# wg-perception/tod

Hardware: AMD Instinct MI355X
Metric: frames/sec @ 640x480, 1M-descriptor DB; achieved HBM GB/s on BF-matcher (higher is better)
Workload: dtype fp4 (+-1) x fp4 -> f32 on the matrix cores (exact integers), f32 in the verifier

## Files before the change

tod_amd/csrc/match_fp4rows.h:

```cpp

__global__ __launch_bounds__(kBlock) void expand_rows_fp4_kernel(const uint32_t* __restrict__ db, uint32_t n_steps, uint4* __restrict__ out) {
  const uint32_t s = blockIdx.x, m = threadIdx.x >> 6, l = threadIdx.x & 63u;
  if (s >= n_steps) return;
  const Fp4Consts kc = fp4_consts();
  const mfma_i32x8 e = expand_word(db[(size_t)fp4_rows_src_row(s, l) * kWords + fp4_rows_src_word(m, l)], kc);
  *reinterpret_cast<uint4*>(reinterpret_cast<char*>(out) + fp4_rows_offset(s, m, l)) =
      uint4{(uint32_t)e[0], (uint32_t)e[1], (uint32_t)e[2], (uint32_t)e[3]};
}
static_assert(kBlock == 256, "expand_rows_fp4_kernel: one workgroup = the 4 x 64 fragments of a step");

typedef uint32_t fp4_u32x4 __attribute__((ext_vector_type(4)));
struct Fp4StepLoader {
  __amdgpu_buffer_rsrc_t copy;
  uint32_t step0, n_steps, lane_off;
  __device__ __forceinline__ Fp4StepLoader(const uint4* p, uint32_t copy_bytes, uint32_t s0, uint32_t n, uint32_t lane)
      : copy(__builtin_amdgcn_make_buffer_rsrc(const_cast<uint4*>(p), 0, (int)copy_bytes, 0x00020000)), step0(s0), n_steps(n),
        lane_off((uint32_t)fp4_rows_offset(0, 0, lane)) {}
  template <bool M_SCALAR>
  __device__ __forceinline__ mfma_i32x8 load(uint32_t step, uint32_t m) const {
    const uint32_t step_off = (uint32_t)fp4_rows_offset(step0 + min(step, n_steps - 1u), M_SCALAR ? m : 0u, 0);
    const fp4_u32x4 v = __builtin_amdgcn_raw_buffer_load_b128(copy, (int)(lane_off + (M_SCALAR ? 0u : m * kFp4FragBytes)), (int)step_off, 0);
    return mfma_i32x8{(int)v.x, (int)v.y, (int)v.z, (int)v.w, 0, 0, 0, 0};
  }
};

template <int K, int SPLIT>
__device__ __forceinline__ void fp4rows_block_test_part(mfma_f32x16& acc, const Fp4Row& rows, const Fp4Row& q, float& thr, float& thrp,
                                                        uint32_t r_lane, uint32_t n_lim, uint32_t (&best)[K], uint32_t& n_pass) {
  if (__builtin_expect(__builtin_amdgcn_ballot_w64(block_reaches<true, false>(acc, thrp)) == 0ull, 1)) return;
  ++n_pass;
#pragma unroll
  for (int s = SPLIT; s < 4; ++s) acc = __builtin_amdgcn_mfma_scale_f32_32x32x64_f8f6f4(rows.s[s], q.s[s], acc, 4, 4, 0, 0, 0, 0);
  mfma_block_test<K, false, true>(acc, thr, r_lane, n_lim, best);
  thrp = thr - 64.f * (float)(4 - SPLIT);
}

template <int N>
struct Fp4Frags { mfma_i32x8 s[N]; };
template <int N>
__device__ __forceinline__ mfma_f32x16 dot_frags(const Fp4Frags<N>& a, const Fp4Frags<N>& b) {
  mfma_f32x16 acc = {0.f, 0.f, 0.f, 0.f, 0.f, 0.f, 0.f, 0.f, 0.f, 0.f, 0.f, 0.f, 0.f, 0.f, 0.f, 0.f};
#pragma unroll
  for (int s = 0; s < N; ++s) acc = __builtin_amdgcn_mfma_scale_f32_32x32x64_f8f6f4(a.s[s], b.s[s], acc, 4, 4, 0, 0, 0, 0);
  return acc;
}
__device__ __forceinline__ uint4 load_query_packed(const uint32_t* __restrict__ q, uint32_t qi, uint32_t nq, uint32_t h) {
  return *reinterpret_cast<const uint4*>(q + (size_t)(qi < nq ? qi : nq - 1u) * kWords + 4u * h);
}
__device__ __forceinline__ uint32_t packed_word(const uint4& p, int m) { return m == 0 ? p.x : m == 1 ? p.y : m == 2 ? p.z : p.w; }

template <int K, int SPLIT>
__device__ __forceinline__ void fp4rows_block_test_part(mfma_f32x16& acc, const Fp4StepLoader& rows, uint32_t own_step,
                                                        const uint32_t* __restrict__ q, uint32_t qi, uint32_t nq, uint32_t h,
                                                        const Fp4Consts& kc, float& thr, float& thrp, uint32_t r_lane, uint32_t n_lim,
                                                        uint32_t (&best)[K], uint32_t& n_pass) {
  if (__builtin_expect(__builtin_amdgcn_ballot_w64(block_reaches<true, false>(acc, thrp)) == 0ull, 1)) return;
  ++n_pass;
  asm volatile("" : "+v"(qi));
  mfma_i32x8 tail[4 - SPLIT];
#pragma unroll
  for (int s = SPLIT; s < 4; ++s) tail[s - SPLIT] = rows.template load<true>(own_step, s);
  const uint4 p = load_query_packed(q, qi, nq, h);
#pragma unroll
  for (int s = SPLIT; s < 4; ++s)
    acc = __builtin_amdgcn_mfma_scale_f32_32x32x64_f8f6f4(tail[s - SPLIT], expand_word(packed_word(p, s), kc), acc, 4, 4, 0, 0, 0, 0);
  mfma_block_test<K, false, true>(acc, thr, r_lane, n_lim, best);
  asm("" : "+v"(thr));
  thrp = thr - 64.f * (float)(4 - SPLIT);
}

template <int K, int QT, bool MASK, bool IMAX, int SPLIT = 0>
__device__ __forceinline__ void fp4rows_step(const Fp4Row& a, Fp4Row& a_next, const Fp4StepLoader& rows, uint32_t next_step,
                                             const Fp4Row (&qb)[QT], float (&thr)[QT], float (&thrp)[QT], uint32_t (&best)[QT][K],
                                             mfma_f32x16& acc_even, mfma_f32x16& acc_odd, uint32_t r_lane, uint32_t n_lim, uint32_t& n_pass) {
  constexpr bool HALF = SPLIT != 0;
  constexpr int kEarly = HALF ? SPLIT : 4;
  static_assert(!(HALF && MASK) && !(HALF && !IMAX) && QT >= 4, "split blocks: unmasked steps, integer maximum; >= 4 query blocks");
  static_assert(SPLIT == 0 || SPLIT == 2 || SPLIT == 3, "2 or 3 of the 4 MFMAs first");
#pragma unroll
  for (int t = 0; t < QT; ++t) {
    if (HALF) { if (t & 1) acc_odd = dot_part0<HALF ? SPLIT : 2>(a, qb[t]); else acc_even = dot_part0<HALF ? SPLIT : 2>(a, qb[t]); }
    else { if (t & 1) acc_odd = dot_block(a, qb[t]); else acc_even = dot_block(a, qb[t]); }
    if (t == 0) {
#pragma unroll
      for (int m = 0; m < kEarly; ++m) a_next.s[m] = rows.template load<!HALF>(next_step, m);
    }
    if (t == 1) {
#pragma unroll
      for (int m = kEarly; m < 4; ++m) a_next.s[m] = rows.template load<!HALF>(next_step, m);
    }
    if (HALF) {
      if (t == 0) fp4rows_block_test_part<K, HALF ? SPLIT : 2>(acc_odd, a_next, qb[QT - 1], thr[QT - 1], thrp[QT - 1], r_lane - 32u, n_lim, best[QT - 1], n_pass);
      else fp4rows_block_test_part<K, HALF ? SPLIT : 2>((t & 1) ? acc_even : acc_odd, a, qb[t - 1], thr[t - 1], thrp[t - 1], r_lane, n_lim, best[t - 1], n_pass);
    } else {
      if (t == 0) mfma_block_test<K, MASK, IMAX>(acc_odd, thr[QT - 1], r_lane - 32u, n_lim, best[QT - 1]);
      else mfma_block_test<K, MASK, IMAX>((t & 1) ? acc_even : acc_odd, thr[t - 1], r_lane, n_lim, best[t - 1]);
    }
  }
}

template <int K, int QT, int SPLIT>
__device__ __forceinline__ void fp4rows_split_step(const Fp4Frags<SPLIT>& a, Fp4Frags<SPLIT>& a_next, const Fp4StepLoader& rows, uint32_t step,
                                                   const Fp4Frags<SPLIT> (&qh)[QT], const uint32_t* __restrict__ q, uint32_t q0c, uint32_t nq,
                                                   uint32_t h, const Fp4Consts& kc, float (&thr)[QT], float (&thrp)[QT],
                                                   uint32_t (&best)[QT][K], mfma_f32x16& acc_even, mfma_f32x16& acc_odd, uint32_t r_lane,
                                                   uint32_t n_lim, uint32_t& n_pass) {
  static_assert(SPLIT == 2 || SPLIT == 3, "2 or 3 of the 4 MFMAs first");
  static_assert(QT >= 4 && QT % 2 == 0, "the pending block alternates between two accumulators");
#pragma unroll
  for (int t = 0; t < QT; ++t) {
    if (t & 1) acc_odd = dot_frags(a, qh[t]); else acc_even = dot_frags(a, qh[t]);
    if (t == 0) {
#pragma unroll
      for (int m = 0; m < SPLIT; ++m) a_next.s[m] = rows.template load<false>(step + 1u, m);
    }
    if (t == 0) fp4rows_block_test_part<K, SPLIT>(acc_odd, rows, step - 1u, q, q0c + 32u * (QT - 1), nq, h, kc, thr[QT - 1], thrp[QT - 1], r_lane - 32u, n_lim, best[QT - 1], n_pass);
    else fp4rows_block_test_part<K, SPLIT>((t & 1) ? acc_even : acc_odd, rows, step, q, q0c + 32u * (t - 1), nq, h, kc, thr[t - 1], thrp[t - 1], r_lane, n_lim, best[t - 1], n_pass);
  }
}

struct PairConsts {
  mfma_f32x16 magic;
  int scale_one, scale_field;
  int bias;
};
__device__ __forceinline__ PairConsts pair_consts(uint32_t cut) {
  PairConsts pk;
  const float m = PairPack::magic(cut);
#pragma unroll
  for (int i = 0; i < 16; ++i) pk.magic[i] = m;
  asm volatile("v_mov_b32 %0, %1" : "=v"(pk.scale_one) : "n"(PairPack::kScaleOne));
  asm volatile("v_mov_b32 %0, %1" : "=v"(pk.scale_field) : "n"(PairPack::kScaleField));
  pk.bias = PairPack::bias(cut);
  return pk;
}
__device__ __forceinline__ void dot_pair(mfma_f32x16& acc, const Fp4Frags<2>& a, const Fp4Frags<2>& qa, const Fp4Frags<2>& qb, const PairConsts& pk) {
  acc = __builtin_amdgcn_mfma_scale_f32_32x32x64_f8f6f4(a.s[0], qa.s[0], pk.magic, 4, 4, 0, 0, 0, 0);
  acc = __builtin_amdgcn_mfma_scale_f32_32x32x64_f8f6f4(a.s[1], qa.s[1], acc, 4, 4, 0, 0, 0, 0);
  acc = __builtin_amdgcn_mfma_scale_f32_32x32x64_f8f6f4(a.s[0], qb.s[0], acc, 4, 4, 0, pk.scale_field, 0, pk.scale_one);
  acc = __builtin_amdgcn_mfma_scale_f32_32x32x64_f8f6f4(a.s[1], qb.s[1], acc, 4, 4, 0, pk.scale_field, 0, pk.scale_one);
  asm volatile("" : "+v"(acc));
}
__device__ __forceinline__ uint32_t pair_or(const mfma_f32x16& acc) {
  uint32_t g[5];
#pragma unroll
  for (int j = 0; j < 5; ++j) {
    g[j] = (uint32_t)__float_as_int(acc[3 * j]) | (uint32_t)__float_as_int(acc[3 * j + 1]) | (uint32_t)__float_as_int(acc[3 * j + 2]);
    asm("" : "+v"(g[j]));
  }
  return (g[0] | g[1] | g[2]) | (g[3] | g[4] | (uint32_t)__float_as_int(acc[15]));
}
template <int K, int FIELD>
__device__ __forceinline__ void fp4rows_pair_complete(const mfma_f32x16& packed, int bias, const Fp4StepLoader& rows, uint32_t own_step,
                                                      const uint32_t* __restrict__ q, uint32_t qi, uint32_t nq, uint32_t h, const Fp4Consts& kc,
                                                      float& thr, uint32_t r_lane, uint32_t n_lim, uint32_t (&best)[K], uint32_t& n_pass) {
  ++n_pass;
  asm volatile("" : "+v"(qi));
  mfma_f32x16 acc;
#pragma unroll
  for (int i = 0; i < 16; ++i) acc[i] = (float)PairPack::unpack((uint32_t)__float_as_int(packed[i]), FIELD, bias);
  mfma_i32x8 tail[2];
#pragma unroll
  for (int s = 2; s < 4; ++s) tail[s - 2] = rows.template load<true>(own_step, s);
  const uint4 p = load_query_packed(q, qi, nq, h);
#pragma unroll
  for (int s = 2; s < 4; ++s)
    acc = __builtin_amdgcn_mfma_scale_f32_32x32x64_f8f6f4(tail[s - 2], expand_word(packed_word(p, s), kc), acc, 4, 4, 0, 0, 0, 0);
  mfma_block_test<K, false, true>(acc, thr, r_lane, n_lim, best);
  asm("" : "+v"(thr));
}
template <int K>
__device__ __forceinline__ void fp4rows_pair_test(const mfma_f32x16& acc, const PairConsts& pk, const Fp4StepLoader& rows, uint32_t own_step,
                                                  const uint32_t* __restrict__ q, uint32_t qi, uint32_t nq, uint32_t h, const Fp4Consts& kc,
                                                  float& thr_a, float& thr_b, uint32_t r_lane, uint32_t n_lim, uint32_t (&best_a)[K],
                                                  uint32_t (&best_b)[K], uint32_t& n_pass) {
  const uint32_t o = pair_or(acc);
  if (__builtin_expect(__builtin_amdgcn_ballot_w64((o & PairPack::kFlagMask) != 0u) == 0ull, 1)) return;
  if (__builtin_amdgcn_ballot_w64((o & PairPack::kFlagA) != 0u) != 0ull)
    fp4rows_pair_complete<K, 0>(acc, pk.bias, rows, own_step, q, qi, nq, h, kc, thr_a, r_lane, n_lim, best_a, n_pass);
  if (__builtin_amdgcn_ballot_w64((o & PairPack::kFlagB) != 0u) != 0ull)
    fp4rows_pair_complete<K, 1>(acc, pk.bias, rows, own_step, q, qi + 32u, nq, h, kc, thr_b, r_lane, n_lim, best_b, n_pass);
}
template <int K, int QT, int PH>
__device__ __forceinline__ void fp4rows_pair_step(const Fp4Frags<2>& a, Fp4Frags<2>& a_next, const Fp4StepLoader& rows, uint32_t step,
                                                  const Fp4Frags<2> (&qh)[QT], const uint32_t* __restrict__ q, uint32_t q0c, uint32_t nq,
                                                  uint32_t h, const Fp4Consts& kc, const PairConsts& pk, float (&thr)[QT],
                                                  uint32_t (&best)[QT][K], mfma_f32x16& acc_even, mfma_f32x16& acc_odd, uint32_t r_lane,
                                                  uint32_t n_lim, uint32_t& n_pass) {
  static_assert(QT >= 4 && QT % 2 == 0, "whole pairs; the pending pair alternates between two accumulators");
  constexpr int NP = QT / 2;
#pragma unroll
  for (int j = 0; j < NP; ++j) {
    const bool odd = ((NP * PH + j) & 1) != 0;
    dot_pair(odd ? acc_odd : acc_even, a, qh[2 * j], qh[2 * j + 1], pk);
    if (j == 0) {
#pragma unroll
      for (int m = 0; m < 2; ++m) a_next.s[m] = rows.template load<false>(step + 1u, m);
    }
    constexpr int kLast = NP - 1;
    if (j == 0) fp4rows_pair_test<K>(odd ? acc_even : acc_odd, pk, rows, step - 1u, q, q0c + 64u * kLast, nq, h, kc, thr[2 * kLast], thr[2 * kLast + 1], r_lane - 32u, n_lim, best[2 * kLast], best[2 * kLast + 1], n_pass);
    else fp4rows_pair_test<K>(odd ? acc_even : acc_odd, pk, rows, step, q, q0c + 64u * (j - 1), nq, h, kc, thr[2 * j - 2], thr[2 * j - 1], r_lane, n_lim, best[2 * j - 2], best[2 * j - 1], n_pass);
  }
}

template <int K, int QT, int SPLIT>
__device__ __forceinline__ void fp4rows_split_masked_step(const Fp4Row& a, const Fp4Frags<SPLIT> (&qh)[QT], const uint32_t (&qtail)[QT][4 - SPLIT],
                                                          const Fp4Consts& kc, float (&thr)[QT], uint32_t (&best)[QT][K],
                                                          mfma_f32x16& acc_even, mfma_f32x16& acc_odd, uint32_t r_lane, uint32_t n_lim) {
#pragma unroll
  for (int t = 0; t < QT; ++t) {
    Fp4Frags<SPLIT> ah;
#pragma unroll
    for (int s = 0; s < SPLIT; ++s) ah.s[s] = a.s[s];
    mfma_f32x16 acc = dot_frags(ah, qh[t]);
#pragma unroll
    for (int s = SPLIT; s < 4; ++s) acc = __builtin_amdgcn_mfma_scale_f32_32x32x64_f8f6f4(a.s[s], expand_word(qtail[t][s - SPLIT], kc), acc, 4, 4, 0, 0, 0, 0);
    if (t & 1) acc_odd = acc; else acc_even = acc;
    if (t == 0) mfma_block_test<K, true, true>(acc_odd, thr[QT - 1], r_lane - 32u, n_lim, best[QT - 1]);
    else mfma_block_test<K, true, true>((t & 1) ? acc_even : acc_odd, thr[t - 1], r_lane, n_lim, best[t - 1]);
  }
}

#ifndef TOD_K4X_STATIC_PRIO
#define TOD_K4X_STATIC_PRIO 1
#endif
template <int K, int QT, int MODE>
__global__ __launch_bounds__(kBlock, 2) void hamming_topk_fp4rows(const uint4* __restrict__ rows_fp4,
                                                                  const uint32_t* __restrict__ q, uint32_t n_rows,
                                                                  uint32_t nq, uint32_t nq_pad, uint32_t rows_per_tile,
                                                                  uint32_t n_tiles, uint32_t n_qw, uint32_t n_qw64,
                                                                  uint32_t blocks_per_xcd, uint32_t tiles_per_xcd, uint32_t cut,
                                                                  uint32_t share_period,
                                                                  uint32_t* __restrict__ part, uint32_t* bound,
                                                                  uint8_t* __restrict__ stored, uint32_t* half_stats) {
  static_assert(QT == 4 || QT == 6, "four or six query blocks per wave: with eight the fragments of two steps do not fit beside them");
  constexpr bool IMAX = MODE >= 1;
  constexpr int HALF = MODE == 4 ? 2 : (MODE >= 2 ? MODE : 0);
  constexpr float kPartOff = HALF ? 64.f * (float)(4 - HALF) : 0.f;
  const uint32_t xcd = blockIdx.x & 7u, slot = blockIdx.x >> 3;
  uint32_t tile, qw;
  if (tiles_per_xcd) {
    const uint32_t local = __builtin_amdgcn_readfirstlane(slot * kWavesPerBlock + (threadIdx.x >> 6));
    if (local >= tiles_per_xcd * n_qw) return;
    tile = xcd * tiles_per_xcd + local / n_qw; qw = local % n_qw;
  } else {
    const uint32_t vblock = xcd * blocks_per_xcd + slot;
    const uint32_t item = __builtin_amdgcn_readfirstlane(vblock * kWavesPerBlock + (threadIdx.x >> 6));
    tile = item / n_qw; qw = item % n_qw;
  }
  if (tile >= n_tiles) return;
  const uint32_t lane = threadIdx.x & 63u, c = lane & 31u, h = lane >> 5;
  const uint32_t q0 = qw * (32u * QT);

  const Fp4Consts kc = fp4_consts();
  constexpr bool TAILS = HALF == 2;
  constexpr bool PAIRS = MODE == 2;
  constexpr int NF = TAILS ? HALF : 4;
  using Frags = typename std::conditional<TAILS, Fp4Frags<NF>, Fp4Row>::type;
  Frags qb[QT];
  uint32_t best[QT][K];
  float thr[QT], thrp[QT];
#pragma unroll
  for (int t = 0; t < QT; ++t) {
    if constexpr (TAILS) {
      const uint4 p = load_query_packed(q, q0 + 32u * t + c, nq, h);
#pragma unroll
      for (int m = 0; m < NF; ++m) qb[t].s[m] = expand_word(packed_word(p, m), kc);
    } else {
      load_query_block(q, q0 + 32u * t + c, nq, h, qb[t], kc);
    }
#pragma unroll
    for (int j = 0; j < K; ++j) best[t][j] = 0xFFFFFFFFu;
    thr[t] = thr_of_limit(cut);
    if constexpr (!PAIRS) thrp[t] = thr[t] - kPartOff;
  }

  const uint32_t row0 = tile * rows_per_tile;
  const uint32_t n_local = min(n_rows, row0 + rows_per_tile) - row0;
  const uint32_t n_full = n_local / 32u, n_steps = (n_local + 31u) / 32u;
  const Fp4StepLoader rows(rows_fp4, (uint32_t)fp4_rows_bytes(n_rows), row0 / 32u, n_steps, lane);
  Frags a0, a1;
#pragma unroll
  for (int m = 0; m < NF; ++m) a0.s[m] = rows.template load<false>(0, m);
  a1 = a0;
  mfma_f32x16 acc_even, acc_odd;
  PairConsts pk;
  if constexpr (PAIRS) { pk = pair_consts(cut); acc_odd = pk.magic; }
  else {
#pragma unroll
    for (int i = 0; i < 16; ++i) acc_odd[i] = kNoBlock;
  }
  uint32_t seen[QT];
#pragma unroll
  for (int t = 0; t < QT; ++t) seen[t] = 0xFFFFFFFFu;
  uint32_t next_share = 2u, step = 0, n_pass = 0;
  if (TOD_K4X_STATIC_PRIO && HALF == 2 && QT == 6 && ((slot >> 5) & 1u)) __builtin_amdgcn_s_setprio(1);
  for (; step + 2u <= n_full; step += 2u) {
    if constexpr (PAIRS) {
      fp4rows_pair_step<K, QT, 0>(a0, a1, rows, step, qb, q, q0 + c, nq, h, kc, pk, thr, best, acc_even, acc_odd, lane_row_base(step, h), n_local, n_pass);
      fp4rows_pair_step<K, QT, 1>(a1, a0, rows, step + 1u, qb, q, q0 + c, nq, h, kc, pk, thr, best, acc_even, acc_odd, lane_row_base(step, h) + 32u, n_local, n_pass);
    } else if constexpr (TAILS) {
      fp4rows_split_step<K, QT, NF>(a0, a1, rows, step, qb, q, q0 + c, nq, h, kc, thr, thrp, best, acc_even, acc_odd, lane_row_base(step, h), n_local, n_pass);
      fp4rows_split_step<K, QT, NF>(a1, a0, rows, step + 1u, qb, q, q0 + c, nq, h, kc, thr, thrp, best, acc_even, acc_odd, lane_row_base(step, h) + 32u, n_local, n_pass);
    } else {
      fp4rows_step<K, QT, false, IMAX, HALF>(a0, a1, rows, step + 1u, qb, thr, thrp, best, acc_even, acc_odd, lane_row_base(step, h), n_local, n_pass);
      fp4rows_step<K, QT, false, IMAX, HALF>(a1, a0, rows, step + 2u, qb, thr, thrp, best, acc_even, acc_odd, lane_row_base(step, h) + 32u, n_local, n_pass);
    }
    if (step + 2u >= next_share) {
      next_share += share_period;
      exchange_bounds<K, QT>(bound, q0, c, nq, best, seen, thr, [](uint32_t limit) { return thr_of_limit(limit); },
                             [&](int t) { if constexpr (!PAIRS) thrp[t] = thr[t] - kPartOff; });
    }
  }
  if constexpr (TAILS) {
    if (step > 0u) {
      if constexpr (PAIRS)
        fp4rows_pair_test<K>(acc_odd, pk, rows, step - 1u, q, q0 + c + 32u * (QT - 2), nq, h, kc, thr[QT - 2], thr[QT - 1], lane_row_base(step - 1u, h), n_local, best[QT - 2], best[QT - 1], n_pass);
      else
        fp4rows_block_test_part<K, NF>(acc_odd, rows, step - 1u, q, q0 + c + 32u * (QT - 1), nq, h, kc, thr[QT - 1], thrp[QT - 1], lane_row_base(step - 1u, h), n_local, best[QT - 1], n_pass);
#pragma unroll
      for (int i = 0; i < 16; ++i) acc_odd[i] = kNoBlock;
      if (lane == 0 && half_stats) { atomicAdd(half_stats, n_pass); atomicAdd(half_stats + 1, step * (uint32_t)QT); }
    }
    if (step < n_steps) {
      uint32_t qtail[QT][4 - NF];
#pragma unroll
      for (int t = 0; t < QT; ++t) {
        const uint4 p = load_query_packed(q, q0 + 32u * t + c, nq, h);
#pragma unroll
        for (int m = NF; m < 4; ++m) qtail[t][m - NF] = packed_word(p, m);
      }
      Fp4Row a, a_next;
#pragma unroll
      for (int m = 0; m < NF; ++m) a.s[m] = a0.s[m];
#pragma unroll
      for (int m = NF; m < 4; ++m) a.s[m] = rows.template load<false>(step, m);
      for (; step < n_steps; ++step) {
#pragma unroll
        for (int m = 0; m < 4; ++m) a_next.s[m] = rows.template load<false>(step + 1u, m);
        fp4rows_split_masked_step<K, QT, NF>(a, qb, qtail, kc, thr, best, acc_even, acc_odd, lane_row_base(step, h), n_local);
        a = a_next;
      }
    }
  } else {
    if (HALF && step > 0u) {
      fp4rows_block_test_part<K, HALF ? HALF : 2>(acc_odd, a1, qb[QT - 1], thr[QT - 1], thrp[QT - 1], lane_row_base(step - 1u, h), n_local, best[QT - 1], n_pass);
#pragma unroll
      for (int i = 0; i < 16; ++i) acc_odd[i] = kNoBlock;
      if (lane == 0 && half_stats) { atomicAdd(half_stats, n_pass); atomicAdd(half_stats + 1, step * (uint32_t)QT); }
    }
    for (; step < n_steps; ++step) {
      fp4rows_step<K, QT, true, IMAX>(a0, a1, rows, step + 1u, qb, thr, thrp, best, acc_even, acc_odd, lane_row_base(step, h), n_local, n_pass);
      a0 = a1;
    }
  }
  mfma_block_test<K, true, IMAX>(acc_odd, thr[QT - 1], lane_row_base(n_steps - 1u, h), n_local, best[QT - 1]);
  store_tile_lists<K, QT>(best, tile, q0, nq, nq_pad, n_qw64, lane, c, h, part, stored);
}
```

Baseline: 23820.

## Move cross-tile bound exchange into rare pair-complete path for PAIRS variant

For the paired-query path, the periodic exchange_bounds call in the main loop is removed. Each query's global bound is instead read and atomically lowered only inside fp4rows_pair_complete, which runs when a candidate passes the packed test. The row-base lane offset is now recomputed there instead of being passed through every step call. This cuts periodic synchronisation and register pressure in the hot loop, at the cost of fresher thresholds arriving only on rare completion events, so pruning may be weaker between events.

```diff
diff --git a/tod_amd/csrc/match_fp4rows.h b/tod_amd/csrc/match_fp4rows.h
--- a/tod_amd/csrc/match_fp4rows.h
+++ b/tod_amd/csrc/match_fp4rows.h
@@ -153,9 +153,13 @@
 template <int K, int FIELD>
 __device__ __forceinline__ void fp4rows_pair_complete(const mfma_f32x16& packed, int bias, const Fp4StepLoader& rows, uint32_t own_step,
                                                       const uint32_t* __restrict__ q, uint32_t qi, uint32_t nq, uint32_t h, const Fp4Consts& kc,
-                                                      float& thr, uint32_t r_lane, uint32_t n_lim, uint32_t (&best)[K], uint32_t& n_pass) {
+                                                      float& thr, uint32_t n_lim, uint32_t (&best)[K], uint32_t& n_pass, uint32_t* bound) {
   ++n_pass;
   asm volatile("" : "+v"(qi));
+  asm volatile("" : "+v"(h));
+  const uint32_t r_lane = lane_row_base(own_step, h);
+  uint32_t* my_bound = bound + (qi < nq ? qi : nq - 1u);
+  const uint32_t seen = __hip_atomic_load(my_bound, __ATOMIC_RELAXED, __HIP_MEMORY_SCOPE_AGENT);
   mfma_f32x16 acc;
 #pragma unroll
   for (int i = 0; i < 16; ++i) acc[i] = (float)PairPack::unpack((uint32_t)__float_as_int(packed[i]), FIELD, bias);
@@ -166,27 +170,30 @@
 #pragma unroll
   for (int s = 2; s < 4; ++s)
     acc = __builtin_amdgcn_mfma_scale_f32_32x32x64_f8f6f4(tail[s - 2], expand_word(packed_word(p, s), kc), acc, 4, 4, 0, 0, 0, 0);
+  if (seen != 0xFFFFFFFFu) thr = fmaxf(thr, thr_of_limit(seen + 1u));
   mfma_block_test<K, false, true>(acc, thr, r_lane, n_lim, best);
+  const uint32_t worst_d = best[K - 1] >> kLocalBits;
+  if (worst_d < kNoLimit && worst_d < seen) atomicMin(my_bound, worst_d);
   asm("" : "+v"(thr));
 }
 template <int K>
 __device__ __forceinline__ void fp4rows_pair_test(const mfma_f32x16& acc, const PairConsts& pk, const Fp4StepLoader& rows, uint32_t own_step,
                                                   const uint32_t* __restrict__ q, uint32_t qi, uint32_t nq, uint32_t h, const Fp4Consts& kc,
-                                                  float& thr_a, float& thr_b, uint32_t r_lane, uint32_t n_lim, uint32_t (&best_a)[K],
-                                                  uint32_t (&best_b)[K], uint32_t& n_pass) {
+                                                  float& thr_a, float& thr_b, uint32_t n_lim, uint32_t (&best_a)[K],
+                                                  uint32_t (&best_b)[K], uint32_t& n_pass, uint32_t* bound) {
   const uint32_t o = pair_or(acc);
   if (__builtin_expect(__builtin_amdgcn_ballot_w64((o & PairPack::kFlagMask) != 0u) == 0ull, 1)) return;
   if (__builtin_amdgcn_ballot_w64((o & PairPack::kFlagA) != 0u) != 0ull)
-    fp4rows_pair_complete<K, 0>(acc, pk.bias, rows, own_step, q, qi, nq, h, kc, thr_a, r_lane, n_lim, best_a, n_pass);
+    fp4rows_pair_complete<K, 0>(acc, pk.bias, rows, own_step, q, qi, nq, h, kc, thr_a, n_lim, best_a, n_pass, bound);
   if (__builtin_amdgcn_ballot_w64((o & PairPack::kFlagB) != 0u) != 0ull)
-    fp4rows_pair_complete<K, 1>(acc, pk.bias, rows, own_step, q, qi + 32u, nq, h, kc, thr_b, r_lane, n_lim, best_b, n_pass);
+    fp4rows_pair_complete<K, 1>(acc, pk.bias, rows, own_step, q, qi + 32u, nq, h, kc, thr_b, n_lim, best_b, n_pass, bound);
 }
 template <int K, int QT, int PH>
 __device__ __forceinline__ void fp4rows_pair_step(const Fp4Frags<2>& a, Fp4Frags<2>& a_next, const Fp4StepLoader& rows, uint32_t step,
                                                   const Fp4Frags<2> (&qh)[QT], const uint32_t* __restrict__ q, uint32_t q0c, uint32_t nq,
                                                   uint32_t h, const Fp4Consts& kc, const PairConsts& pk, float (&thr)[QT],
-                                                  uint32_t (&best)[QT][K], mfma_f32x16& acc_even, mfma_f32x16& acc_odd, uint32_t r_lane,
-                                                  uint32_t n_lim, uint32_t& n_pass) {
+                                                  uint32_t (&best)[QT][K], mfma_f32x16& acc_even, mfma_f32x16& acc_odd,
+                                                  uint32_t n_lim, uint32_t& n_pass, uint32_t* bound) {
   static_assert(QT >= 4 && QT % 2 == 0, "whole pairs; the pending pair alternates between two accumulators");
   constexpr int NP = QT / 2;
 #pragma unroll
@@ -198,8 +205,8 @@
       for (int m = 0; m < 2; ++m) a_next.s[m] = rows.template load<false>(step + 1u, m);
     }
     constexpr int kLast = NP - 1;
-    if (j == 0) fp4rows_pair_test<K>(odd ? acc_even : acc_odd, pk, rows, step - 1u, q, q0c + 64u * kLast, nq, h, kc, thr[2 * kLast], thr[2 * kLast + 1], r_lane - 32u, n_lim, best[2 * kLast], best[2 * kLast + 1], n_pass);
-    else fp4rows_pair_test<K>(odd ? acc_even : acc_odd, pk, rows, step, q, q0c + 64u * (j - 1), nq, h, kc, thr[2 * j - 2], thr[2 * j - 1], r_lane, n_lim, best[2 * j - 2], best[2 * j - 1], n_pass);
+    if (j == 0) fp4rows_pair_test<K>(odd ? acc_even : acc_odd, pk, rows, step - 1u, q, q0c + 64u * kLast, nq, h, kc, thr[2 * kLast], thr[2 * kLast + 1], n_lim, best[2 * kLast], best[2 * kLast + 1], n_pass, bound);
+    else fp4rows_pair_test<K>(odd ? acc_even : acc_odd, pk, rows, step, q, q0c + 64u * (j - 1), nq, h, kc, thr[2 * j - 2], thr[2 * j - 1], n_lim, best[2 * j - 2], best[2 * j - 1], n_pass, bound);
   }
 }
 
@@ -290,15 +297,17 @@
 #pragma unroll
     for (int i = 0; i < 16; ++i) acc_odd[i] = kNoBlock;
   }
-  uint32_t seen[QT];
-#pragma unroll
-  for (int t = 0; t < QT; ++t) seen[t] = 0xFFFFFFFFu;
-  uint32_t next_share = 2u, step = 0, n_pass = 0;
+  [[maybe_unused]] uint32_t seen[QT], next_share = 2u;
+  if constexpr (!PAIRS) {
+#pragma unroll
+    for (int t = 0; t < QT; ++t) seen[t] = 0xFFFFFFFFu;
+  }
+  uint32_t step = 0, n_pass = 0;
   if (TOD_K4X_STATIC_PRIO && HALF == 2 && QT == 6 && ((slot >> 5) & 1u)) __builtin_amdgcn_s_setprio(1);
   for (; step + 2u <= n_full; step += 2u) {
     if constexpr (PAIRS) {
-      fp4rows_pair_step<K, QT, 0>(a0, a1, rows, step, qb, q, q0 + c, nq, h, kc, pk, thr, best, acc_even, acc_odd, lane_row_base(step, h), n_local, n_pass);
-      fp4rows_pair_step<K, QT, 1>(a1, a0, rows, step + 1u, qb, q, q0 + c, nq, h, kc, pk, thr, best, acc_even, acc_odd, lane_row_base(step, h) + 32u, n_local, n_pass);
+      fp4rows_pair_step<K, QT, 0>(a0, a1, rows, step, qb, q, q0 + c, nq, h, kc, pk, thr, best, acc_even, acc_odd, n_local, n_pass, bound);
+      fp4rows_pair_step<K, QT, 1>(a1, a0, rows, step + 1u, qb, q, q0 + c, nq, h, kc, pk, thr, best, acc_even, acc_odd, n_local, n_pass, bound);
     } else if constexpr (TAILS) {
       fp4rows_split_step<K, QT, NF>(a0, a1, rows, step, qb, q, q0 + c, nq, h, kc, thr, thrp, best, acc_even, acc_odd, lane_row_base(step, h), n_local, n_pass);
       fp4rows_split_step<K, QT, NF>(a1, a0, rows, step + 1u, qb, q, q0 + c, nq, h, kc, thr, thrp, best, acc_even, acc_odd, lane_row_base(step, h) + 32u, n_local, n_pass);
@@ -306,16 +315,18 @@
       fp4rows_step<K, QT, false, IMAX, HALF>(a0, a1, rows, step + 1u, qb, thr, thrp, best, acc_even, acc_odd, lane_row_base(step, h), n_local, n_pass);
       fp4rows_step<K, QT, false, IMAX, HALF>(a1, a0, rows, step + 2u, qb, thr, thrp, best, acc_even, acc_odd, lane_row_base(step, h) + 32u, n_local, n_pass);
     }
-    if (step + 2u >= next_share) {
-      next_share += share_period;
-      exchange_bounds<K, QT>(bound, q0, c, nq, best, seen, thr, [](uint32_t limit) { return thr_of_limit(limit); },
-                             [&](int t) { if constexpr (!PAIRS) thrp[t] = thr[t] - kPartOff; });
+    if constexpr (!PAIRS) {
+      if (step + 2u >= next_share) {
+        next_share += share_period;
+        exchange_bounds<K, QT>(bound, q0, c, nq, best, seen, thr, [](uint32_t limit) { return thr_of_limit(limit); },
+                               [&](int t) { thrp[t] = thr[t] - kPartOff; });
+      }
     }
   }
   if constexpr (TAILS) {
     if (step > 0u) {
       if constexpr (PAIRS)
-        fp4rows_pair_test<K>(acc_odd, pk, rows, step - 1u, q, q0 + c + 32u * (QT - 2), nq, h, kc, thr[QT - 2], thr[QT - 1], lane_row_base(step - 1u, h), n_local, best[QT - 2], best[QT - 1], n_pass);
+        fp4rows_pair_test<K>(acc_odd, pk, rows, step - 1u, q, q0 + c + 32u * (QT - 2), nq, h, kc, thr[QT - 2], thr[QT - 1], n_local, best[QT - 2], best[QT - 1], n_pass, bound);
       else
         fp4rows_block_test_part<K, NF>(acc_odd, rows, step - 1u, q, q0 + c + 32u * (QT - 1), nq, h, kc, thr[QT - 1], thrp[QT - 1], lane_row_base(step - 1u, h), n_local, best[QT - 1], n_pass);
 #pragma unroll
```

After: 24970, median of 6. 4.8% higher.
